# AlexGr5/StereoVision

Hardware: AMD Instinct MI355X
Metric: disparity frames/sec + HBM GB/s, 1920x1080 D=128 win=9, 1/2/4/8 GPU (higher is better)
Workload: dtype u8

## Files before the change

stereovision_amd/csrc/sv_capi.cpp:

```cpp
#include "sv_ctx.h"

namespace {
thread_local std::string g_err;
}

namespace svc {

int fail(int code, const std::string& msg) {
    g_err = msg;
    return code;
}

int hipfail(int e, const char* what) {
    return fail(SV_EHIP, std::string(what) + ": " + hipGetErrorString((hipError_t)e));
}

const std::string& last_error_msg() { return g_err; }

int check_image(const void* a, int H, int W) {
    if (!a || H <= 0 || W <= 0) return fail(SV_EINVAL, "null image or non-positive size");
    return 0;
}

int check_match(int H, int W, int min_disp, int num_disp, int win, int cost, sv::MatchPlan* plan) {
// ... 3 lines not shown
    if (min_disp < -4096 || min_disp > 4096) return fail(SV_EINVAL, "min_disp out of range");
    if (cost == SV_COST_SGBM) return 0;
    int rc = sv::plan_match(num_disp, win, cost, plan);
    if (rc == -34) return fail(SV_ERANGE, "cost range too large for the argmin key");
    if (rc != 0) return fail(SV_EINVAL, "unsupported (num_disp, win, cost)");
    return 0;
}

SgbmParams sgbm_reference_params(int win) {
    return {8 * 3 * win * win, 32 * 3 * win * win, 1, 63, 10, 100, 32};
}

int enqueue_speckles(sv_ctx* c, int16_t* d_img, int H, int W, int pitch, int new_val, int max_speckle_size,
                     int max_diff, hipStream_t s, int nf, long long fimg) {
    if (max_speckle_size <= 0) return 0;
    const size_t n = (size_t)H * W * (nf < 1 ? 1 : nf);
    SV_HIP(c->cc_parent.ensure(n * 4));
    SV_HIP(c->cc_size.ensure(n * 4));
    SV_LAUNCH(c, SV_K_SPECKLE, s,
              sv::launch_speckles(d_img, H, W, pitch, new_val, max_speckle_size, max_diff, c->cc_parent.as<int>(),
                                  c->cc_size.as<int>(), s, nf < 1 ? 1 : nf, fimg));
    return 0;
}

constexpr int kSgbmChunk = 32;
size_t sgbm_budget(int device) {
    static const long long env_gb = [] {
        const char* e = std::getenv("SV_SGBM_BUDGET_GB");
        return e ? std::atoll(e) : 0LL;
    }();
    if (env_gb > 0) return (size_t)env_gb << 30;
    size_t fr = 0, tot = 0;
    (void)device;
    if (hipMemGetInfo(&fr, &tot) != hipSuccess || fr == 0) return (size_t)8 << 30;
    return std::min<size_t>(fr / 4, (size_t)48 << 30);
}

int enqueue_sgbm(sv_ctx* c, const uint8_t* L, const uint8_t* R, int H, int W, int pitch, int min_disp,
                 int num_disp, int win, SgbmParams p, int16_t* out, int opitch, hipStream_t s, int nf,
                 long long fs_in, long long fs_out) {
    if (nf < 1) nf = 1;
    if (sv::sgbm_dp(num_disp) < 0) return fail(SV_EINVAL, "num_disp must be in [1, 512]");
    if (W > 16384) return fail(SV_EINVAL, "SGBM: width beyond 16384");
    if (p.P1 < 0 || p.P2 < 0) return fail(SV_EINVAL, "negative P1/P2");
    if (p.P2 <= p.P1) p.P2 = p.P1 + 1;
    if (p.P2 >= 349525) return fail(SV_ERANGE, "SGBM: P2 too large for the 32-bit argmin key");
    p.cap = (p.cap > 15 ? p.cap : 15) | 1;
    if (p.cap > 127) return fail(SV_EINVAL, "preFilterCap must be <= 127");
    sv::SgbmArgs a{};
    a.L = L;
    a.R = R;
    a.H = H;
    a.W = W;
    a.pitch = pitch;
    a.minD = min_disp;
    a.D = num_disp;
// ... 57 lines not shown
        const int n = std::min(chunk, nf - z0);
        a.L = L + z0 * fs_in;
        a.R = R + z0 * fs_in;
        a.out = out + z0 * fs_out;
        SV_LAUNCH(c, SV_K_SGBM, s, sv::launch_sgbm(a, n, s, c->sg_aux, c->sg_ev[0], c->sg_ev[1]));
        const int rc = enqueue_speckles(c, a.out, H, W, opitch, (min_disp - 1) * 16, p.speckle_win,
                                        16 * p.speckle_range, s, n, fs_out);
        if (rc) return rc;
    }
    return 0;
}

int enqueue_disparity(sv_ctx* c, const uint8_t* L, const uint8_t* R, int H, int W, int pitch,
                      int min_disp, int num_disp, int win, int cost, int row0, int row1,
                      int16_t* out, int opitch, hipStream_t s, int nf, long long fs_in,
                      long long fs_out) {
    sv::MatchPlan plan;
    int rc = check_match(H, W, min_disp, num_disp, win, cost, &plan);
    if (rc) return rc;
    if (row0 < 0) row0 = 0;
    if (row1 > H) row1 = H;
    if (row1 <= row0) return 0;
    if (cost == SV_COST_SGBM) {
        if (row0 != 0 || row1 != H) return fail(SV_EINVAL, "SGBM cannot compute a row band (use frames)");
        return enqueue_sgbm(c, L, R, H, W, pitch, min_disp, num_disp, win, sgbm_reference_params(win), out, opitch,
                            s, nf, fs_in, fs_out);
    }
    sv::MatchParams a{};
    a.L = L;
    a.R = R;
    a.H = H;
    a.W = W;
    a.pitch = pitch;
    a.minD = min_disp;
    a.D = num_disp;
    a.win = win;
    a.r = cost == SV_COST_HOG ? 0 : win / 2;
// ... 22 lines not shown
        SV_HIP(c->hog[0].ensure(hb));
        SV_HIP(c->hog[1].ensure(hb));
        SV_LAUNCH(c, SV_K_HOG, s,
                  sv::launch_hog_hist_pairs(L, R, H, W, pitch, win, row0, row1, c->hog[0].as<uint16_t>(),
                                            c->hog[1].as<uint16_t>(), a.nf, a.nf > 1 ? fs_in : 0, fh, s));
        a.HL = c->hog[0].as<uint16_t>();
        a.HR = c->hog[1].as<uint16_t>();
        a.fs_hist = a.nf > 1 ? fh : 0;
    }
    if (sv::ring_split(cost, win, num_disp) && a.X1 > a.X0) {
        const long long ke = sv::ring_split_elems(a.nf, fs_out, row1, opitch);
        SV_HIP(c->keys.ensure((size_t)(2 * ke) * sizeof(uint32_t)));
        a.keys = c->keys.as<uint32_t>();
        a.keys_stride = ke;
    }
    SV_LAUNCH(c, SV_K_MATCH, s, sv::launch_match(a, plan, cost, s));
    return 0;
}

int attach_lut(sv_ctx* c, sv::PostParams& pp, hipStream_t s, bool whole) {
    pp.lut_n = 0;
    pp.lut_shift = 0;
    if (pp.mode == SV_POST_NONE || pp.num_disp <= 0 || pp.num_disp > 512) return 0;
    sv_ctx::LutKey k;
    k.mode = pp.mode;
    k.min_disp = pp.min_disp;
    k.num_disp = pp.num_disp;
    k.m0 = (pp.min_disp - 1) * 16;
    k.n = whole ? pp.num_disp + 1 : (pp.num_disp + 1) * 16;
    k.minf = pp.minf;
    k.maxf = pp.maxf;
    k.rangef = pp.rangef;
    k.mdg = pp.min_disp_global;
    DevBuf& buf = whole ? c->lutw : c->lut;
    sv_ctx::LutKey& key = whole ? c->lutw_key : c->lut_key;
    hipEvent_t& ev = whole ? c->lutw_ev : c->lut_ev;
    hipStream_t& bs = whole ? c->lutw_stream : c->lut_stream;
    const size_t n = (size_t)k.n;
    float* la = buf.as<float>();
    if (!(k == key) || !ev) {
        SV_HIP(buf.ensure(n * (2 * sizeof(float) + 1)));
        la = buf.as<float>();
        if (!ev) SV_HIP(hipEventCreateWithFlags(&ev, hipEventDisableTiming));
        int e = sv::launch_post_lut(pp, k.m0, k.n, whole ? 16 : 1, la, reinterpret_cast<uint8_t*>(la + 2 * n), la + n,
                                    s);
        if (e) return hipfail(e, "launch_post_lut");
        SV_HIP(hipEventRecord(ev, s));
        key = k;
        bs = s;
    } else if (s != bs) {
        SV_HIP(hipStreamWaitEvent(s, ev, 0));
    }
    pp.lut_a = la;
    pp.lut_b = la + n;
    pp.lut_u8 = reinterpret_cast<const uint8_t*>(la + 2 * n);
    pp.lut_m0 = k.m0;
    pp.lut_n = k.n;
    pp.lut_shift = whole ? 4 : 0;
    return 0;
}

int attach_cmap(sv_ctx* c, sv::PostParams& pp, const uint8_t* table, uint8_t* d_bgr, hipStream_t s) {
    pp.out_bgr = nullptr;
    pp.cmap = nullptr;
    if (!d_bgr) return 0;
    if (!table) return fail(SV_EINVAL, "colormap output without a table");
    SV_HIP(c->cmap.ensure(256 * sizeof(uint32_t)));
    if (!c->cmap_valid || std::memcmp(c->cmap_host, table, 768) != 0) {
        uint32_t packed[256];
        for (int i = 0; i < 256; ++i)
            packed[i] = (uint32_t)table[3 * i] | ((uint32_t)table[3 * i + 1] << 8) | ((uint32_t)table[3 * i + 2] << 16);
        SV_HIP(hipMemcpyAsync(c->cmap.p, packed, sizeof(packed), hipMemcpyHostToDevice, s));
        SV_HIP(hipStreamSynchronize(s));
// ... 275 lines not shown
    SV_ENTER(c);
    if (slot < 0 || slot >= 16 || !c->wev[slot]) return fail(SV_EINVAL, "event slot never recorded");
    SV_HIP(hipStreamWaitEvent(pick(c, stream), c->wev[slot], 0));
    return 0;
}

int sv_release_scratch(sv_ctx* c) {
    SV_ENTER(c);
    SV_HIP(hipStreamSynchronize(c->stream));
    if (c->sg_aux) SV_HIP(hipStreamSynchronize(c->sg_aux));
    DevBuf* bufs[] = {&c->img[0], &c->img[1], &c->gray[0], &c->gray[1], &c->d16, &c->fa, &c->fb, &c->fc,
                      &c->u8, &c->harris, &c->hog[0], &c->hog[1], &c->fin, &c->sg_hsum, &c->sg_c,
                      &c->sg_l, &c->sg_lt, &c->sg_band, &c->sg_rec, &c->cc_parent, &c->cc_size, &c->m16,
                      &c->gm16, &c->keys};
    for (auto* b : bufs) b->release();
    return 0;
}

int sv_synchronize(sv_ctx* c) {
    SV_ENTER(c);
    SV_HIP(hipStreamSynchronize(c->stream));
    return 0;
}

void* sv_stream(sv_ctx* c) { return c ? static_cast<void*>(c->stream) : nullptr; }

int sv_plan(int num_disp, int win, int cost, int* dpl, int* lpg, int* lds_bytes) {
    sv::MatchPlan p;
    int rc = sv::plan_match(num_disp, win, cost, &p);
    if (rc == -34) return fail(SV_ERANGE, "cost range too large for the argmin key");
// ... 121 lines not shown
```

stereovision_amd/csrc/sv_capi_dev.cpp:

```cpp
#include "sv_ctx.h"

extern "C" {

int sv_gray_dev(sv_ctx* c, const uint8_t* d_bgr, int H, int W, int pitch, uint8_t* d_gray, void* stream) {
    SV_ENTER(c);
    if (check_image(d_bgr, H, W) || !d_gray) return fail(SV_EINVAL, "bad gray arguments");
    hipStream_t s = pick(c, stream);
    SV_LAUNCH(c, SV_K_GRAY, s, sv::launch_gray(d_bgr, H, W, pitch, d_gray, s));
    return 0;
}

int sv_disparity_dev(sv_ctx* c, const uint8_t* d_left, const uint8_t* d_right, int H, int W, int pitch,
                     int min_disp, int num_disp, int win, int cost, int row0, int row1, int16_t* d_disp16,
                     int out_pitch, void* stream) {
    SV_ENTER(c);
    if (check_image(d_left, H, W) || check_image(d_right, H, W) || !d_disp16)
        return fail(SV_EINVAL, "bad disparity arguments");
    if (pitch < W || out_pitch < W) return fail(SV_EINVAL, "pitch smaller than width");
    hipStream_t s = pick(c, stream);
    SV_SCRATCH(c, s);
    return enqueue_disparity(c, d_left, d_right, H, W, pitch, min_disp, num_disp, win, cost, row0, row1,
                             d_disp16, out_pitch, s);
}

// ... 68 lines not shown
    if (median && out->harris && check_image(d_left, H, W)) return fail(SV_EINVAL, "Harris needs the left frames");
    if (pitch < W) return fail(SV_EINVAL, "pitch smaller than width");
    if (n_frames > 1 && frame_stride < (int64_t)pitch * H) return fail(SV_EINVAL, "frame stride smaller than a frame");
    if ((long long)H * W >= (1LL << 30)) return fail(SV_EINVAL, "frame too large for the median kernel");
    if (n_frames == 0) return 0;
    hipStream_t s = pick(c, stream);
    SV_SCRATCH(c, s);
    const long long fs = (long long)H * W;
    int16_t* d16 = d_disp16;
    if (!d16) {
        SV_HIP(c->d16.ensure((size_t)n_frames * fs * sizeof(int16_t)));
        d16 = c->d16.as<int16_t>();
    }
    if (match) {
        const int rc = enqueue_disparity(c, d_left, d_right, H, W, pitch, min_disp, num_disp, win, cost, 0, H, d16, W,
                                         s, n_frames, frame_stride, fs);
        if (rc) return rc;
    }
    if (!median) return 0;
    sv::PostParams pp;
    float* disp = nullptr;
    int rc = map_out_post(c, out, min_disp, num_disp, cost, true, s, &pp, &disp);
    if (rc) return rc;
    const long long fin = n_frames > 1 ? frame_stride : 0;
    if (out->harris && (W < 8 || H < 8)) {
        SV_LAUNCH(c, SV_K_MEDIAN, s, sv::launch_median_i16(d16, H, W, 0, H, disp, pp, s, n_frames, fs, fs));
        SV_LAUNCH(c, SV_K_HARRIS, s, sv::launch_harris(d_left, H, W, pitch, out->harris, s, n_frames, fin, fs));
        return 0;
    }
    sv::HarrisParams hp{d_left, pitch, fin, out->harris, fs, 0, 0};
    SV_LAUNCH(c, SV_K_MEDIAN, s,
              sv::launch_median_i16(d16, H, W, 0, H, disp, pp, s, n_frames, fs, fs, out->harris ? &hp : nullptr));
    return 0;
}

int sv_harris_dev(sv_ctx* c, const uint8_t* d_gray, int H, int W, int pitch, float* d_out, void* stream) {
    SV_ENTER(c);
    if (check_image(d_gray, H, W) || !d_out) return fail(SV_EINVAL, "bad harris arguments");
// ... 990 lines not shown
    SV_ENTER(c);
    if (!d_img || H <= 0 || W <= 0 || pitch < W) return fail(SV_EINVAL, "bad speckle-filter arguments");
    hipStream_t s = pick(c, stream);
    SV_SCRATCH(c, s);
    return enqueue_speckles(c, d_img, H, W, pitch, new_val, max_speckle_size, max_diff, s);
}

int sv_filter_speckles(sv_ctx* c, int16_t* img, int H, int W, int new_val, int max_speckle_size, int max_diff) {
    SV_ENTER(c);
    SV_SCRATCH(c, c->stream);
    if (!img || H <= 0 || W <= 0) return fail(SV_EINVAL, "bad speckle-filter arguments");
    const size_t bytes = (size_t)H * W * sizeof(int16_t);
    SV_HIP(c->d16.ensure(bytes));
    SV_HIP(c->hin.ensure(bytes));
    std::memcpy(c->hin.p, img, bytes);
    SV_HIP(hipMemcpyAsync(c->d16.p, c->hin.p, bytes, hipMemcpyHostToDevice, c->stream));
    const int rc = enqueue_speckles(c, c->d16.as<int16_t>(), H, W, W, new_val, max_speckle_size, max_diff, c->stream);
    if (rc) return rc;
    Out o[] = {{img, c->d16.p, bytes}};
    return collect(c, o, 1);
}


}
```

stereovision_amd/csrc/sv_ctx.h:

```cpp
#pragma once
#include <cstdio>
#include <cstdlib>
#include <algorithm>
#include <chrono>
#include <cstring>
#include <map>
#include <mutex>
#include <thread>
#include <new>
#include <string>
#include <vector>

#include "sv_internal.h"
#include "sv_pool.h"
#include "../../include/stereovision_amd.h"

namespace svc {
int fail(int code, const std::string& msg);
int hipfail(int e, const char* what);
const std::string& last_error_msg();
}
using svc::fail;
using svc::hipfail;

// ... 5 lines not shown

#define SV_LAUNCH(ctx, kid, stream, call)                          \
    do {                                                           \
        (ctx)->prof_begin((kid), (stream));                        \
        int e_ = (call);                                           \
        if (e_ != 0) {                                             \
            (ctx)->prof_abort();                                   \
            return hipfail(e_, #call);                             \
        }                                                          \
        (ctx)->prof_end((stream));                                 \
    } while (0)

struct DevBuf {
    void* p = nullptr;
    size_t cap = 0;
    hipError_t ensure(size_t n) {
        if (n <= cap) return hipSuccess;
        if (p) (void)hipFree(p);
        p = nullptr;
        cap = 0;
        hipError_t e = hipMalloc(&p, n);
        if (e == hipSuccess) cap = n;
        return e;
    }
    void release() {
        if (p) (void)hipFree(p);
        p = nullptr;
        cap = 0;
    }
    hipError_t ensure_zeroed(size_t n) {
        if (n <= cap) return hipSuccess;
        hipError_t e = ensure(n);
        if (e == hipSuccess) e = hipMemset(p, 0, cap);
        if (e == hipSuccess) e = hipDeviceSynchronize();
        return e;
    }
    template <class T> T* as() const { return static_cast<T*>(p); }
};

struct HostBuf {
// ... 52 lines not shown
        bool operator==(const LutKey& o) const {
            return mode == o.mode && min_disp == o.min_disp && num_disp == o.num_disp && m0 == o.m0 &&
                   n == o.n && std::memcmp(&minf, &o.minf, sizeof(float)) == 0 &&
                   std::memcmp(&maxf, &o.maxf, sizeof(float)) == 0 &&
                   std::memcmp(&rangef, &o.rangef, sizeof(float)) == 0 &&
                   std::memcmp(&mdg, &o.mdg, sizeof(float)) == 0;
        }
    } lut_key, hl_key;
    hipEvent_t lut_ev = nullptr;
    hipStream_t lut_stream = nullptr;
    DevBuf lutw;
    LutKey lutw_key;
    hipEvent_t lutw_ev = nullptr;
    hipStream_t lutw_stream = nullptr;
    HostBuf hin, hout;
    hipStream_t scr_stream = nullptr;
    hipEvent_t scr_ev = nullptr;
    hipEvent_t xev = nullptr;
    hipEvent_t sev = nullptr;
    hipEvent_t gev = nullptr;
    hipEvent_t wev[16] = {};
    bool prof = false;
    std::vector<EvPair> pending;
    std::vector<hipEvent_t> pool;
    double acc_ms[SV_NKERNELS] = {};
    long long cnt[SV_NKERNELS] = {};
    EvPair cur{};
    bool cur_open = false;
    EvPair region{};
    bool region_open = false;
// ... 62 lines not shown
struct SgbmParams {
    int P1, P2, disp12, cap, uniq, speckle_win, speckle_range;
};
SgbmParams sgbm_reference_params(int win);

int check_image(const void* a, int H, int W);
int check_match(int H, int W, int min_disp, int num_disp, int win, int cost, sv::MatchPlan* plan);
int enqueue_speckles(sv_ctx* c, int16_t* d_img, int H, int W, int pitch, int new_val, int max_speckle_size,
                     int max_diff, hipStream_t s, int nf = 1, long long fimg = 0);
int enqueue_sgbm(sv_ctx* c, const uint8_t* L, const uint8_t* R, int H, int W, int pitch, int min_disp,
                 int num_disp, int win, SgbmParams p, int16_t* out, int opitch, hipStream_t s, int nf = 1,
                 long long fs_in = 0, long long fs_out = 0);
int enqueue_disparity(sv_ctx* c, const uint8_t* L, const uint8_t* R, int H, int W, int pitch,
                      int min_disp, int num_disp, int win, int cost, int row0, int row1,
                      int16_t* out, int opitch, hipStream_t s, int nf = 1, long long fs_in = 0,
                      long long fs_out = 0);
int attach_lut(sv_ctx* c, sv::PostParams& pp, hipStream_t s, bool whole = false);
int attach_cmap(sv_ctx* c, sv::PostParams& pp, const uint8_t* table, uint8_t* d_bgr, hipStream_t s);
sv::PostParams make_post(int mode, float minf, float maxf, float rangef, float mdg, int min_disp,
                         int num_disp, float* a, uint8_t* u8, float* b);

int map_out_post(sv_ctx* c, const sv_map_out* out, int min_disp, int num_disp, int cost, bool allow_harris,
                 hipStream_t s, sv::PostParams* pp, float** disp);

struct MapOut {
    int fmt = 0;
    void* map = nullptr;
    int d8_base = 0;
    size_t el() const { return fmt == SV_MAP_D8 ? 1 : 2; }
};
int check_map(int fmt, const void* map, int cost, int num_disp);
// ... 57 lines not shown
```

stereovision_amd/csrc/sv_image.hip:

```cpp
#include <cstdlib>
#include <cstring>
#include <type_traits>
#include "sv_internal.h"
#include "sv_median_net.h"

namespace sv {
namespace {

__device__ __forceinline__ int clampi(int v, int lo, int hi) { return min(max(v, lo), hi); }
__device__ __forceinline__ int refl101(int i, int n) {
    if (n == 1) return 0;
    i = i < 0 ? -i : i;
    return i >= n ? 2 * (n - 1) - i : i;
}

__global__ void k_gray(const uint8_t* __restrict__ bgr, int H, int W, int pitch,
                       uint8_t* __restrict__ gray) {
    const int x = blockIdx.x * blockDim.x + threadIdx.x;
    const int y = blockIdx.y;
    if (x >= W) return;
    const uint8_t* p = bgr + (size_t)y * pitch + 3 * x;
    const int v = p[0] * 1868 + p[1] * 9617 + p[2] * 4899 + (1 << 13);
    gray[(size_t)y * W + x] = (uint8_t)(v >> 14);
}
// ... 619 lines not shown
    return *reinterpret_cast<T*>(reinterpret_cast<B*>(base) + (uint32_t)(i * (uint32_t)sizeof(T)));
}

__device__ __forceinline__ PostVals post_median(const PostParams& pp, int mv) {
    const uint32_t dm = (uint32_t)(mv - pp.lut_m0);
    const uint32_t li = dm >> pp.lut_shift;
    if (li < (uint32_t)pp.lut_n && (dm & ((1u << pp.lut_shift) - 1u)) == 0) {
        PostVals o;
        o.a = at(pp.lut_a, li);
        o.u = at(pp.lut_u8, li);
        o.b = pp.mode == POST_SCALED ? at(pp.lut_b, li) : 0.0f;
        return o;
    }
    return post_vals(pp, (float)mv / 16.0f);
}

__global__ __launch_bounds__(256) void k_post_m16(const int16_t* __restrict__ in, long long n,
                                                  float* __restrict__ disp, PostParams pp) {
    const long long i0 = ((long long)blockIdx.x * 256 + threadIdx.x) * 8;
    if (i0 >= n) return;
    const bool vec = i0 + 8 <= n && ((((uintptr_t)in) & 15) | (((uintptr_t)disp | (uintptr_t)pp.out_a |
                                                                  (uintptr_t)pp.out_b) & 15) |
                                     ((uintptr_t)pp.out_u8 & 7)) == 0;
    if (vec) {
        const uint4 raw = *reinterpret_cast<const uint4*>(in + i0);
        const uint32_t w[4] = {raw.x, raw.y, raw.z, raw.w};
        int mv[8];
#pragma unroll
        for (int q = 0; q < 4; ++q) {
            mv[2 * q] = (int)(int16_t)(w[q] & 0xFFFFu);
// ... 21 lines not shown
            b[1] = make_float4(o[4].b, o[5].b, o[6].b, o[7].b);
        }
        return;
    }
    for (long long i = i0; i < i0 + 8 && i < n; ++i) {
        const int mv = (int)in[i];
        if (disp) disp[i] = (float)mv / 16.0f;
        if (pp.mode == POST_NONE) continue;
        const PostVals o = post_median(pp, mv);
        pp.out_a[i] = o.a;
        pp.out_u8[i] = o.u;
        if (pp.mode == POST_SCALED) pp.out_b[i] = o.b;
    }
}

template <int HF>
__global__ __launch_bounds__(256) void k_median_i16(const int16_t* __restrict__ in, int H, int W,
                                                    int row0, int row1, float* __restrict__ disp,
                                                    PostParams pp, long long fs_in, long long fs_out,
                                                    HarrisParams hp) {
    if (HF != 0 && (int)blockIdx.x >= hp.mbx) {
        const int w = (int)(blockIdx.x - hp.mbx) * 4 + (int)(threadIdx.x >> 6);
        const int y0 = row0 + (int)blockIdx.y * MQ_H;
        if constexpr (HF == 2) {
            const int x0 = w * 248;
            if (x0 < W && y0 < row1)
                harris_wave4<MQ_H, 4>(hp.g + blockIdx.z * hp.fs_in, H, W, hp.pitch, hp.out + blockIdx.z * hp.fs_out,
                                      x0, y0, threadIdx.x & 63);
        } else {
            const int x0 = w * 60;
            if (x0 < W && y0 < row1)
// ... 146 lines not shown
            for (int i = 0; i < 5; ++i) r = __builtin_elementwise_min(r, __builtin_elementwise_max(cw[w][i], u[4 - i]));
            m[w] = r;
        }
        const uint32_t a0 = __builtin_bit_cast(uint32_t, m[0]), a1 = __builtin_bit_cast(uint32_t, m[1]);
        mp[h] = (a0 & 0xFFFFu) | (a1 << 16);
        mp[h + 2] = (a0 >> 16) | (a1 & 0xFFFF0000u);
    }
    static_assert(sizeof(srt) >= MQ_H * (MQ_W / 2) * sizeof(uint32_t), "med must fit in srt");
    auto med = reinterpret_cast<uint32_t (*)[MQ_W / 2]>(&srt[0][0][0]);
    __syncthreads();
    med[tb][tx >> 1] = mp[0];
    med[tb + 1][tx >> 1] = mp[1];
    med[tb + 2][tx >> 1] = mp[2];
    med[tb + 3][tx >> 1] = mp[3];
    __syncthreads();
#pragma unroll
    for (int pass = 0; pass < 2; ++pass) {
        const int r = (int)(threadIdx.x >> 5) + 8 * pass, c4 = (int)(threadIdx.x & 31) * 4;
        const int y = y0 + r, x = x0 + c4;
        if (y >= row1 || x >= W) continue;
        const uint2 raw = *reinterpret_cast<const uint2*>(&med[r][c4 >> 1]);
        const int mv[4] = {(int)(int16_t)(raw.x & 0xFFFF), (int)(int16_t)(raw.x >> 16),
                           (int)(int16_t)(raw.y & 0xFFFF), (int)(int16_t)(raw.y >> 16)};
        const uint32_t i = (uint32_t)y * W + x;
        const bool vec = x + 3 < W && (W & 3) == 0 &&
                         (((uintptr_t)disp | (uintptr_t)pp.out_a | (uintptr_t)pp.out_b) & 15) == 0 &&
                         (((uintptr_t)pp.out_u8 | (uintptr_t)pp.out_bgr | (uintptr_t)pp.out_d8) & 3) == 0 &&
                         ((uintptr_t)pp.out_m16 & 7) == 0;
        if (vec) {
            if (disp)
                at(reinterpret_cast<float4*>(disp), i >> 2) =
                    make_float4((float)mv[0] / 16.0f, (float)mv[1] / 16.0f, (float)mv[2] / 16.0f, (float)mv[3] / 16.0f);
            if (pp.out_m16) at(reinterpret_cast<uint2*>(pp.out_m16), i >> 2) = raw;
            if (pp.out_d8)
                at(reinterpret_cast<uint32_t*>(pp.out_d8), i >> 2) =
                    (uint32_t)(uint8_t)((mv[0] >> 4) - pp.d8_base) | ((uint32_t)(uint8_t)((mv[1] >> 4) - pp.d8_base) << 8) |
                    ((uint32_t)(uint8_t)((mv[2] >> 4) - pp.d8_base) << 16) |
                    ((uint32_t)(uint8_t)((mv[3] >> 4) - pp.d8_base) << 24);
            if (pp.mode == POST_NONE) continue;
            PostVals o[4];
#pragma unroll
            for (int q = 0; q < 4; ++q) o[q] = post_median(pp, mv[q]);
            at(reinterpret_cast<float4*>(pp.out_a), i >> 2) = make_float4(o[0].a, o[1].a, o[2].a, o[3].a);
            at(reinterpret_cast<uint32_t*>(pp.out_u8), i >> 2) =
                (uint32_t)o[0].u | ((uint32_t)o[1].u << 8) | ((uint32_t)o[2].u << 16) | ((uint32_t)o[3].u << 24);
            if (pp.mode == POST_SCALED)
                at(reinterpret_cast<float4*>(pp.out_b), i >> 2) = make_float4(o[0].b, o[1].b, o[2].b, o[3].b);
            if (pp.out_bgr) {
                const uint32_t c0 = pp.cmap[o[0].u], c1 = pp.cmap[o[1].u], c2 = pp.cmap[o[2].u],
                               c3 = pp.cmap[o[3].u];
                uint32_t* d = &at(reinterpret_cast<uint32_t*>(pp.out_bgr), 3 * (i >> 2));
                d[0] = c0 | (c1 << 24);
                d[1] = (c1 >> 8) | (c2 << 16);
                d[2] = (c2 >> 16) | (c3 << 8);
            }
            continue;
        }
#pragma unroll
        for (int q = 0; q < 4; ++q) {
            if (x + q >= W) break;
            if (disp) at(disp, i + q) = (float)mv[q] / 16.0f;
            if (pp.out_m16) at(pp.out_m16, i + q) = (int16_t)mv[q];
            if (pp.out_d8) at(pp.out_d8, i + q) = (uint8_t)((mv[q] >> 4) - pp.d8_base);
            if (pp.mode == POST_NONE) continue;
            const PostVals o = post_median(pp, mv[q]);
            at(pp.out_a, i + q) = o.a;
            at(pp.out_u8, i + q) = o.u;
            if (pp.mode == POST_SCALED) at(pp.out_b, i + q) = o.b;
            if (pp.out_bgr) {
                const uint32_t c = pp.cmap[o.u];
                uint8_t* d = &at(pp.out_bgr, 3 * (i + q));
                d[0] = (uint8_t)c;
                d[1] = (uint8_t)(c >> 8);
                d[2] = (uint8_t)(c >> 16);
            }
        }
    }
}

__global__ __launch_bounds__(256) void k_median_f32(const float* __restrict__ in, int H, int W,
// ... 142 lines not shown
    if (row1 <= row0 || nf <= 0) return 0;
    if ((long long)H * W >= (1LL << 30)) return (int)hipErrorInvalidValue;
    HarrisParams hp{};
    hp.mbx = (W + MQ_W - 1) / MQ_W;
    int hbx = 0;
    if (harris && harris->g) {
        hp = *harris;
        hp.mbx = (W + MQ_W - 1) / MQ_W;
        static const bool med4 = [] {
            const char* e = std::getenv("SV_HARRIS_MED4");
            return !(e && e[0] == '0');
        }();
        hp.form = (med4 && W >= 256) ? 1 : 0;
        hbx = hp.form ? ((W + 247) / 248 + 3) / 4 : ((W + 59) / 60 + 3) / 4;
    }
    void (*fn)(const int16_t*, int, int, int, int, float*, PostParams, long long, long long, HarrisParams) =
        hbx == 0 ? k_median_i16<0> : hp.form ? k_median_i16<2> : k_median_i16<1>;
    hipLaunchKernelGGL(fn, dim3(hp.mbx + hbx, (row1 - row0 + MQ_H - 1) / MQ_H, nf),
                       dim3(256), 0, s, in, H, W, row0, row1, disp, pp, fs_in, fs_out, hp);
    return (int)hipGetLastError();
}

int launch_post_m16(const int16_t* in, long long n, float* disp, const PostParams& pp, hipStream_t s) {
    if (n <= 0) return 0;
    const long long blocks = (n + 8 * 256 - 1) / (8 * 256);
    if (blocks > 0x7FFFFFFFLL) return (int)hipErrorInvalidValue;
    hipLaunchKernelGGL(k_post_m16, dim3((unsigned)blocks), dim3(256), 0, s, in, n, disp, pp);
    return (int)hipGetLastError();
}

int launch_median_f32(const float* in, int H, int W, float* out, hipStream_t s) {
    hipLaunchKernelGGL(k_median_f32, dim3((W + MT_W - 1) / MT_W, (H + MT_H - 1) / MT_H), dim3(256),
// ... 26 lines not shown
```

stereovision_amd/csrc/sv_internal.h:

```cpp
#pragma once
#include <hip/hip_runtime.h>
#include <stdint.h>

#include <string>

struct sv_comm;

namespace sv {

__device__ __forceinline__ void sad_u32_acc(uint32_t& a, uint32_t b, uint32_t c) {
    asm("v_sad_u32 %0, %0, %1, %2" : "+v"(a) : "v"(b), "v"(c));
}

int set_error(int code, const std::string& msg);

int comm_group_start();
int comm_group_end();
int comm_send(sv_comm* c, const void* buf, size_t bytes, int peer, hipStream_t s);
int comm_recv(sv_comm* c, void* buf, size_t bytes, int peer, hipStream_t s);
int comm_rank(const sv_comm* c);
int comm_size(const sv_comm* c);
int comm_device(const sv_comm* c);

enum Cost { COST_SAD = 0, COST_SSD = 1, COST_HOG = 2, COST_SGBM = 3 };
// ... 15 lines not shown
    int minD, D, r;
    int win;
    int X0, X1;
    int row0, row1;
    int lpg, lpg_log2, dbits;
    int16_t* out;
    int opitch;
    int nf;
    long long fs_in, fs_out, fs_hist;
    uint32_t pad_key;
    int segm;
    unsigned* work_ctr;
    int xcd_map;
    uint32_t* keys;
    long long keys_stride;
};

int plan_match(int num_disp, int win, int cost, MatchPlan* plan);
uint64_t max_cost(int win, int cost);
size_t match_lds_bytes(const MatchPlan& p, int r, int cost);
int launch_match(const MatchParams& a, const MatchPlan& p, int cost, hipStream_t s);
bool ring_split(int cost, int win, int num_disp);
bool ring_ssd(int cost, int win, int num_disp);
bool ssd_mfma(int cost, int win, int num_disp);
bool ssd_mfma_fits(const MatchParams& a, int cost);
int launch_ssd_mfma(const MatchParams& a, hipStream_t s);
long long ring_split_elems(int nf, long long fs_out, int row1, int opitch);
int launch_fill_i16(int16_t* out, int opitch, int H, int W, int16_t v, hipStream_t s);

int launch_gray(const uint8_t* bgr, int H, int W, int pitch, uint8_t* gray, hipStream_t s);
// ... 116 lines not shown
    float minf, maxf, rangef, min_disp_global;
    int min_disp, num_disp;
    float* out_a;
    uint8_t* out_u8;
    float* out_b;
    uint8_t* out_bgr;
    const uint32_t* cmap;
    int16_t* out_m16;
    uint8_t* out_d8;
    int d8_base;
    const float* lut_a;
    const uint8_t* lut_u8;
    const float* lut_b;
    int lut_m0, lut_n;
    int lut_shift;
};
struct HarrisParams {
    const uint8_t* g;
    int pitch;
    long long fs_in;
    float* out;
    long long fs_out;
    int mbx;
    int form;
};
int launch_median_i16(const int16_t* in, int H, int W, int row0, int row1, float* disp,
                      const PostParams& pp, hipStream_t s, int nf = 1, long long fs_in = 0,
                      long long fs_out = 0, const HarrisParams* harris = nullptr);
int launch_median_f32(const float* in, int H, int W, float* out, hipStream_t s);
int launch_post_m16(const int16_t* in, long long n, float* disp, const PostParams& pp, hipStream_t s);
int launch_post(const float* disp, int n, const PostParams& pp, hipStream_t s);
// ... 5 lines not shown
```

stereovision_amd/csrc/sv_match.hip:

```cpp
#include "sv_internal.h"
#include "sv_xcd.h"

#include <algorithm>
#include <cstdlib>
#include <vector>
#include <cstdio>
#include <type_traits>

namespace sv {
namespace {

constexpr int COST_SAD4 = 4;

__host__ __device__ __forceinline__ int seg_width(int lpg, int dpl, int sm = 4) { return (sm * lpg + dpl - 1) / dpl * dpl; }
__host__ __device__ __forceinline__ int wave_cols(int lpg, int dpl, int sm = 4) { return (64 / lpg) * seg_width(lpg, dpl, sm); }
int seg_mult(int kind, int r) {
    static const int sm4 = [] {
        const char* e = std::getenv("SV_SAD4_SEG");
        const int v = e ? std::atoi(e) : 0;
        return v >= 1 && v <= 8 ? v : 0;
    }();
    if (kind != COST_SAD4) return 4;
    if (sm4) return sm4;
    return (2 * r - 2 + 3) / 4 <= 2 ? 4 : 2;
// ... 162 lines not shown
__device__ __forceinline__ void transpose4(uint32_t a, uint32_t b, uint32_t c, uint32_t d, uint32_t (&o)[4]) {
    const uint32_t t0 = __builtin_amdgcn_perm(b, a, 0x05010400u);
    const uint32_t t1 = __builtin_amdgcn_perm(b, a, 0x07030602u);
    const uint32_t t2 = __builtin_amdgcn_perm(d, c, 0x05010400u);
    const uint32_t t3 = __builtin_amdgcn_perm(d, c, 0x07030602u);
    o[0] = __builtin_amdgcn_perm(t2, t0, 0x05040100u);
    o[1] = __builtin_amdgcn_perm(t2, t0, 0x07060302u);
    o[2] = __builtin_amdgcn_perm(t3, t1, 0x05040100u);
    o[3] = __builtin_amdgcn_perm(t3, t1, 0x07060302u);
}

template <int R>
__device__ __forceinline__ void sad4_group_words(const uint32_t (&rw)[2 * R + 4],
                                                 uint32_t (&w)[PackCfg<COST_SAD4, R>::NW][4]) {
    constexpr int NC = PackCfg<COST_SAD4, R>::NW - 4, NCR = 2 * R - 2;
#pragma unroll
    for (int m = 0; m < NC; ++m) {
        uint32_t d[4];
#pragma unroll
        for (int t = 0; t < 4; ++t) d[t] = 4 * m + t < NCR ? rw[3 + 4 * m + t] : 0u;
        transpose4(d[0], d[1], d[2], d[3], w[m]);
    }
#pragma unroll
    for (int q = 0; q < 4; ++q) {
        uint32_t d[3];
        int n = 0;
#pragma unroll
        for (int j = q; j <= 2; ++j) d[n++] = rw[j];
#pragma unroll
        for (int j = 2 * R + 1; j <= 2 * R + q; ++j) d[n++] = rw[j];
        transpose4(d[0], d[1], d[2], 0u, w[NC + q]);
    }
}

template <int COST, int ND>
__device__ __forceinline__ void build_group(const MatchParams& a, const uint8_t* img, int cg, int y,
                                            uint32_t (&w)[PackCfg<COST, ND>::NW][4]) {
    const int r = COST == COST_SAD4 ? ND : a.r;
    auto row = [&](int j) -> uint32_t {
        const int yy = clampi(y - r + j, 0, a.H - 1);
        return *reinterpret_cast<const uint32_t*>(img + (size_t)yy * a.pitch + cg);
    };
    if constexpr (COST == COST_SAD4) {
        uint32_t rw[2 * ND + 4];
#pragma unroll
        for (int j = 0; j < 2 * ND + 4; ++j) rw[j] = row(j);
// ... 56 lines not shown
                for (int i = 0; i < 8; ++i) v[i] = i < NW ? w[i < NW ? i : 0][k] : 0u;
                put<COST, ND>(base + (right ? rslot(idx, c0, DPL) : idx), v);
            }
        } else {
#pragma unroll
            for (int k = 0; k < 4; ++k) {
                const int idx = cg + k - cfirst;
                if (idx < 0 || idx >= n) continue;
                build_pack<COST, ND>(a, img, nullptr, cg + k, y, base + (right ? rslot(idx, c0, DPL) : idx));
            }
        }
    }
    }
}

template <int R, int MF, int DPL>
__device__ __forceinline__ void build_ring_packs(const MatchParams& a, int y, int cL0, int NL, int cR0,
                                                 int NRlog, int c0, PackOut<COST_SAD4, R> Lp,
                                                 PackOut<COST_SAD4, R> Rp, int lane) {
    constexpr int NW = PackCfg<COST_SAD4, R>::NW, NRW = 2 * R + 4;
    const bool aligned = ((reinterpret_cast<uintptr_t>(a.L) | reinterpret_cast<uintptr_t>(a.R) |
                           (uintptr_t)a.pitch) & 3u) == 0;
    const bool near = (long long)a.H * (long long)a.pitch < 0x7FFFFFFFLL;
    if (!aligned || !near) {
        build_all_packs<COST_SAD4, R, DPL>(a, y, cL0, NL, cR0, NRlog, c0, Lp, Rp, lane);
        return;
    }
    const auto lsrc = __builtin_amdgcn_make_buffer_rsrc(const_cast<uint8_t*>(a.L), 0, 0x7FFFFFFF, 0x00020000);
    const auto rsrc = __builtin_amdgcn_make_buffer_rsrc(const_cast<uint8_t*>(a.R), 0, 0x7FFFFFFF, 0x00020000);
    const int aL = cL0 & ~3, aR = cR0 & ~3;
    const int gL = (cL0 + NL - aL + 3) >> 2, gR = (cR0 + NRlog - aR + 3) >> 2;
    const int G = gL + gR;
    int roff[NRW];
#pragma unroll
    for (int j = 0; j < NRW; ++j) roff[j] = clampi(y - R + j, 0, a.H - 1) * a.pitch;
    for (int g0 = 0; g0 < G; g0 += 64 * MF) {
        uint32_t rw[MF][NRW];
#pragma unroll
        for (int m = 0; m < MF; ++m) {
            const int gi = g0 + lane + 64 * m;
            const bool right = gi >= gL;
            const int cg = right ? aR + 4 * (gi - gL) : aL + 4 * gi;
            const bool in = gi < G && cg >= 0 && cg + 4 <= a.W;
            if (in && !right) {
#pragma unroll
                for (int j = 0; j < NRW; ++j) rw[m][j] = __builtin_amdgcn_raw_buffer_load_b32(lsrc, cg, roff[j], 0);
            }
            if (in && right) {
#pragma unroll
                for (int j = 0; j < NRW; ++j) rw[m][j] = __builtin_amdgcn_raw_buffer_load_b32(rsrc, cg, roff[j], 0);
            }
        }
#pragma unroll
        for (int m = 0; m < MF; ++m) {
            const int gi = g0 + lane + 64 * m;
            if (gi >= G) continue;
            const bool right = gi >= gL;
            const int cg = right ? aR + 4 * (gi - gL) : aL + 4 * gi;
            const int cfirst = right ? cR0 : cL0, n = right ? NRlog : NL;
            const PackOut<COST_SAD4, R> base = right ? Rp : Lp;
            if (cg >= 0 && cg + 4 <= a.W) {
                uint32_t w[NW][4];
                sad4_group_words<R>(rw[m], w);
#pragma unroll
                for (int k = 0; k < 4; ++k) {
                    const int idx = cg + k - cfirst;
                    if (idx < 0 || idx >= n) continue;
                    uint32_t v[8];
#pragma unroll
                    for (int i = 0; i < 8; ++i) v[i] = i < NW ? w[i < NW ? i : 0][k] : 0u;
                    put<COST_SAD4, R>(base + (right ? rslot(idx, c0, DPL) : idx), v);
                }
            } else {
#pragma unroll
                for (int k = 0; k < 4; ++k) {
                    const int idx = cg + k - cfirst;
                    if (idx < 0 || idx >= n) continue;
                    build_pack<COST_SAD4, R>(a, right ? a.R : a.L, nullptr, cg + k, y,
                                             base + (right ? rslot(idx, c0, DPL) : idx));
                }
            }
        }
    }
}

template <int COST, int ND, int DPL>
// ... 357 lines not shown
    constexpr int LPG = LPGT;
    const int S = a.segm;
    const int WC = (64 / LPG) * S;
    constexpr bool SADU = PK || R <= 5;
    constexpr int M = SADU ? W2 + 1 : W2;
    constexpr int U = M % 4 == 0 ? M : M % 2 == 0 ? 2 * M : 4 * M;
    constexpr int NCH = U / 4;
    const int Tn = (S + 2 * R + 3) & ~3;
    const int nit = (Tn + U - 1) / U;
    const int e0 = (nit * U - Tn) >> 2;
    const int NL = WC - S + Tn + 1;
    const int NRlog = WC - S + Tn + 4 * LPG;
    constexpr int c0 = 1;
    const int NRphys = NRlog + (NRlog + c0) / RG_DPL + 1;
    uint4* wbase = smem + (LDSMIN ? RING_SCRATCH_BYTES / 16 : 0);
    typename P::CT* cbase = reinterpret_cast<typename P::CT*>(wbase + (size_t)(NL + NRphys));
    const PackOut<COST_SAD4, R> Lw{wbase, cbase};
    const PackOut<COST_SAD4, R> Rw{wbase + NL, cbase + NL};
    const PackPtr<COST_SAD4, R> Lp{Lw.x, Lw.c};
    const PackPtr<COST_SAD4, R> Rp{Rw.x, Rw.c};

    const int y = a.row0 + by * 4;
    const int yc = min(y, a.row1 - 1);
    const int xw = a.X0 + bx * WC;
    const int cL0 = xw - R;
    const int cR0 = cL0 - a.minD - (4 * LPG - 1);
    build_ring_packs<R, 3, RG_DPL>(a, yc, cL0, NL, cR0, NRlog, c0, Lw, Rw, lane);

    if (!KEYS && bx == 0) {
        const int16_t inv = (int16_t)((a.minD - 1) * 16);
#pragma unroll
        for (int q = 0; q < 4; ++q) {
            if (y + q >= a.row1) break;
            int16_t* orow = a.out + (size_t)(y + q) * a.opitch;
            for (int x = lane; x < a.X0; x += 64) orow[x] = inv;
            for (int x = a.X1 + lane; x < a.W; x += 64) orow[x] = inv;
        }
    }
    __syncthreads();
    if (y >= a.row1) return;

    const int g = lane / LPG;
    const int l = lane & (LPG - 1);
    const int xs = xw + g * S;
// ... 362 lines not shown
    const int G = 64 / lpg;
    int best = 8;
    long long best_cost = -1;
    for (int S = 8; S <= 1024; S += 4) {
        if (S > 8 && ring_lds_bytes(lpg, S, r, ldsmin) > 20 * 1024) break;
        const long long cost = (long long)((band + G * S - 1) / (G * S)) * ((S + 2 * r + 3) & ~3);
        if (best_cost < 0 || cost <= best_cost) { best = S; best_cost = cost; }
    }
    return best;
}
size_t ring_lds_bytes(int lpg, int seg, int r, bool ldsmin) {
    const int wc = (64 / lpg) * seg;
    const int tn = (seg + 2 * r + 3) & ~3;
    const int nl = wc - seg + tn + 1, nr = wc - seg + tn + 4 * lpg;
    const int nrp = nr + (nr + 1) / RG_DPL + 1;
    return (size_t)(nl + nrp) * (r <= 3 ? 20 : r <= 5 ? 24 : 28) + (ldsmin ? RING_SCRATCH_BYTES : 0);
}

template <int R, int LPG, bool KEYS, bool SSD>
int launch_ring_rl(const MatchParams& a, size_t lds, hipStream_t s) {
    static const bool defer = [] {
        const char* e = std::getenv("SV_RING_DEFER");
        return !(e && e[0] == '0');
    }();
    void (*fn)(MatchParams);
    if constexpr (SSD) fn = k_match_ring<R, LPG, R != 5, false, true>;
    else if constexpr (KEYS) fn = k_match_ring<R, LPG, R != 5, true>;
    else fn = (defer && R != 5) ? k_match_ring<R, LPG, R != 5, false> : k_match_ring<R, LPG, false, false>;
    if constexpr (R == 4 && LPG == 32 && !KEYS && !SSD) {
        if (ring_ldsmin(LPG, R, KEYS, SSD)) fn = k_match_ring<R, LPG, false, false, false, true>;
    }
// ... 213 lines not shown
```

Baseline: 31770.

## Skip repeated margin fills, use unchecked whole LUT, and streamline ring pack building

Tracks whether the invalid-disparity margins of the internal d16 buffer were already written, keyed on buffer identity, generation and geometry. When the key matches, the ring match kernel skips refilling those margins. The median kernel gains a whole-LUT variant that masks the index instead of range checking, backed by a padded LUT allocation, and its vector-store check is hoisted out of the loop. The SAD4 word transpose is rebuilt with byte-permute instructions, and right-ring slot stores use a computed base with padded LDS. The risks are stale margins if another writer reaches d16 without invalidating the key, and slightly more LDS per block.

```diff
diff --git a/stereovision_amd/csrc/sv_capi.cpp b/stereovision_amd/csrc/sv_capi.cpp
--- a/stereovision_amd/csrc/sv_capi.cpp
+++ b/stereovision_amd/csrc/sv_capi.cpp
@@ -41,6 +41,7 @@
 int enqueue_speckles(sv_ctx* c, int16_t* d_img, int H, int W, int pitch, int new_val, int max_speckle_size,
                      int max_diff, hipStream_t s, int nf, long long fimg) {
     if (max_speckle_size <= 0) return 0;
+    c->scratch_written(d_img);
     const size_t n = (size_t)H * W * (nf < 1 ? 1 : nf);
     SV_HIP(c->cc_parent.ensure(n * 4));
     SV_HIP(c->cc_size.ensure(n * 4));
@@ -67,6 +68,7 @@
                  int num_disp, int win, SgbmParams p, int16_t* out, int opitch, hipStream_t s, int nf,
                  long long fs_in, long long fs_out) {
     if (nf < 1) nf = 1;
+    c->scratch_written(out);
     if (sv::sgbm_dp(num_disp) < 0) return fail(SV_EINVAL, "num_disp must be in [1, 512]");
     if (W > 16384) return fail(SV_EINVAL, "SGBM: width beyond 16384");
     if (p.P1 < 0 || p.P2 < 0) return fail(SV_EINVAL, "negative P1/P2");
@@ -154,13 +156,15 @@
 int enqueue_disparity(sv_ctx* c, const uint8_t* L, const uint8_t* R, int H, int W, int pitch,
                       int min_disp, int num_disp, int win, int cost, int row0, int row1,
                       int16_t* out, int opitch, hipStream_t s, int nf, long long fs_in,
-                      long long fs_out) {
+                      long long fs_out, bool track_margins) {
     sv::MatchPlan plan;
     int rc = check_match(H, W, min_disp, num_disp, win, cost, &plan);
     if (rc) return rc;
     if (row0 < 0) row0 = 0;
     if (row1 > H) row1 = H;
     if (row1 <= row0) return 0;
+    const sv_ctx::MarginKey had = c->d16_margins;
+    c->scratch_written(out);
     if (cost == SV_COST_SGBM) {
         if (row0 != 0 || row1 != H) return fail(SV_EINVAL, "SGBM cannot compute a row band (use frames)");
         return enqueue_sgbm(c, L, R, H, W, pitch, min_disp, num_disp, win, sgbm_reference_params(win), out, opitch,
@@ -213,13 +217,31 @@
         a.keys = c->keys.as<uint32_t>();
         a.keys_stride = ke;
     }
+    sv_ctx::MarginKey key;
+    if (track_margins && out == c->d16.as<int16_t>() && row0 == 0 && row1 == H) {
+        key.valid = true;
+        key.p = c->d16.p;
+        key.gen = c->d16.gen;
+        key.H = H;
+        key.W = W;
+        key.opitch = opitch;
+        key.X0 = a.X0;
+        key.X1 = a.X1;
+        key.min_disp = min_disp;
+        key.nf = a.nf;
+        key.fs_out = fs_out;
+        a.margins_done = had.covers(key) ? 1 : 0;
+        if (a.margins_done) key = had;
+    }
     SV_LAUNCH(c, SV_K_MATCH, s, sv::launch_match(a, plan, cost, s));
+    if (key.valid) c->d16_margins = key;
     return 0;
 }
 
 int attach_lut(sv_ctx* c, sv::PostParams& pp, hipStream_t s, bool whole) {
     pp.lut_n = 0;
     pp.lut_shift = 0;
+    pp.lut_cap = 0;
     if (pp.mode == SV_POST_NONE || pp.num_disp <= 0 || pp.num_disp > 512) return 0;
     sv_ctx::LutKey k;
     k.mode = pp.mode;
@@ -238,7 +260,7 @@
     const size_t n = (size_t)k.n;
     float* la = buf.as<float>();
     if (!(k == key) || !ev) {
-        SV_HIP(buf.ensure(n * (2 * sizeof(float) + 1)));
+        SV_HIP(buf.ensure(whole ? (n + sv::kLutWholeSpan) * 2 * sizeof(float) : n * (2 * sizeof(float) + 1)));
         la = buf.as<float>();
         if (!ev) SV_HIP(hipEventCreateWithFlags(&ev, hipEventDisableTiming));
         int e = sv::launch_post_lut(pp, k.m0, k.n, whole ? 16 : 1, la, reinterpret_cast<uint8_t*>(la + 2 * n), la + n,
@@ -256,6 +278,7 @@
     pp.lut_m0 = k.m0;
     pp.lut_n = k.n;
     pp.lut_shift = whole ? 4 : 0;
+    pp.lut_cap = whole ? k.n + sv::kLutWholeSpan : k.n;
     return 0;
 }
 
@@ -561,6 +584,7 @@
                       &c->sg_l, &c->sg_lt, &c->sg_band, &c->sg_rec, &c->cc_parent, &c->cc_size, &c->m16,
                       &c->gm16, &c->keys};
     for (auto* b : bufs) b->release();
+    c->d16_margins.valid = false;
     return 0;
 }
 
diff --git a/stereovision_amd/csrc/sv_capi_dev.cpp b/stereovision_amd/csrc/sv_capi_dev.cpp
--- a/stereovision_amd/csrc/sv_capi_dev.cpp
+++ b/stereovision_amd/csrc/sv_capi_dev.cpp
@@ -106,7 +106,7 @@
     }
     if (match) {
         const int rc = enqueue_disparity(c, d_left, d_right, H, W, pitch, min_disp, num_disp, win, cost, 0, H, d16, W,
-                                         s, n_frames, frame_stride, fs);
+                                         s, n_frames, frame_stride, fs, !d_disp16);
         if (rc) return rc;
     }
     if (!median) return 0;
@@ -114,6 +114,8 @@
     float* disp = nullptr;
     int rc = map_out_post(c, out, min_disp, num_disp, cost, true, s, &pp, &disp);
     if (rc) return rc;
+    pp.lut_unchecked = match && cost != SV_COST_SGBM && pp.lut_shift == 4 && pp.lut_m0 == (min_disp - 1) * 16 &&
+                       pp.lut_n == num_disp + 1;
     const long long fin = n_frames > 1 ? frame_stride : 0;
     if (out->harris && (W < 8 || H < 8)) {
         SV_LAUNCH(c, SV_K_MEDIAN, s, sv::launch_median_i16(d16, H, W, 0, H, disp, pp, s, n_frames, fs, fs));
@@ -1134,6 +1136,7 @@
     SV_HIP(c->d16.ensure(bytes));
     SV_HIP(c->hin.ensure(bytes));
     std::memcpy(c->hin.p, img, bytes);
+    c->scratch_written(c->d16.p);
     SV_HIP(hipMemcpyAsync(c->d16.p, c->hin.p, bytes, hipMemcpyHostToDevice, c->stream));
     const int rc = enqueue_speckles(c, c->d16.as<int16_t>(), H, W, W, new_val, max_speckle_size, max_diff, c->stream);
     if (rc) return rc;
diff --git a/stereovision_amd/csrc/sv_ctx.h b/stereovision_amd/csrc/sv_ctx.h
--- a/stereovision_amd/csrc/sv_ctx.h
+++ b/stereovision_amd/csrc/sv_ctx.h
@@ -43,8 +43,10 @@
 struct DevBuf {
     void* p = nullptr;
     size_t cap = 0;
+    unsigned long long gen = 0;
     hipError_t ensure(size_t n) {
         if (n <= cap) return hipSuccess;
+        ++gen;
         if (p) (void)hipFree(p);
         p = nullptr;
         cap = 0;
@@ -53,6 +55,7 @@
         return e;
     }
     void release() {
+        ++gen;
         if (p) (void)hipFree(p);
         p = nullptr;
         cap = 0;
@@ -135,6 +138,23 @@
     hipEvent_t lutw_ev = nullptr;
     hipStream_t lutw_stream = nullptr;
     HostBuf hin, hout;
+    struct MarginKey {
+        bool valid = false;
+        const void* p = nullptr;
+        unsigned long long gen = 0;
+        int H = 0, W = 0, opitch = 0, X0 = 0, X1 = 0, min_disp = 0, nf = 0;
+        long long fs_out = 0;
+        bool covers(const MarginKey& o) const {
+            return valid && p == o.p && gen == o.gen && H == o.H && W == o.W && opitch == o.opitch &&
+                   X0 == o.X0 && X1 == o.X1 && min_disp == o.min_disp && nf >= o.nf &&
+                   (o.nf <= 1 || fs_out == o.fs_out);
+        }
+    } d16_margins;
+    void scratch_written(const void* out) {
+        const char* b = static_cast<const char*>(d16.p);
+        const char* o = static_cast<const char*>(out);
+        if (b && o >= b && o < b + d16.cap) d16_margins.valid = false;
+    }
     hipStream_t scr_stream = nullptr;
     hipEvent_t scr_ev = nullptr;
     hipEvent_t xev = nullptr;
@@ -227,7 +247,7 @@
 int enqueue_disparity(sv_ctx* c, const uint8_t* L, const uint8_t* R, int H, int W, int pitch,
                       int min_disp, int num_disp, int win, int cost, int row0, int row1,
                       int16_t* out, int opitch, hipStream_t s, int nf = 1, long long fs_in = 0,
-                      long long fs_out = 0);
+                      long long fs_out = 0, bool track_margins = false);
 int attach_lut(sv_ctx* c, sv::PostParams& pp, hipStream_t s, bool whole = false);
 int attach_cmap(sv_ctx* c, sv::PostParams& pp, const uint8_t* table, uint8_t* d_bgr, hipStream_t s);
 sv::PostParams make_post(int mode, float minf, float maxf, float rangef, float mdg, int min_disp,
diff --git a/stereovision_amd/csrc/sv_image.hip b/stereovision_amd/csrc/sv_image.hip
--- a/stereovision_amd/csrc/sv_image.hip
+++ b/stereovision_amd/csrc/sv_image.hip
@@ -657,6 +657,14 @@
     }
     return post_vals(pp, (float)mv / 16.0f);
 }
+__device__ __forceinline__ PostVals post_median_whole(const PostParams& pp, int mv) {
+    const uint32_t li = ((uint32_t)(mv - pp.lut_m0) >> 4) & (uint32_t)(kLutWholeSpan - 1);
+    PostVals o;
+    o.a = at(pp.lut_a, li);
+    o.u = at(pp.lut_u8, li);
+    o.b = pp.mode == POST_SCALED ? at(pp.lut_b, li) : 0.0f;
+    return o;
+}
 
 __global__ __launch_bounds__(256) void k_post_m16(const int16_t* __restrict__ in, long long n,
                                                   float* __restrict__ disp, PostParams pp) {
@@ -708,7 +716,7 @@
     }
 }
 
-template <int HF>
+template <int HF, bool WH>
 __global__ __launch_bounds__(256) void k_median_i16(const int16_t* __restrict__ in, int H, int W,
                                                     int row0, int row1, float* __restrict__ disp,
                                                     PostParams pp, long long fs_in, long long fs_out,
@@ -885,6 +893,11 @@
     med[tb + 2][tx >> 1] = mp[2];
     med[tb + 3][tx >> 1] = mp[3];
     __syncthreads();
+    auto post = [&](int mv) { return WH ? post_median_whole(pp, mv) : post_median(pp, mv); };
+    const bool vec = (W & 3) == 0 &&
+                     (((uintptr_t)disp | (uintptr_t)pp.out_a | (uintptr_t)pp.out_b) & 15) == 0 &&
+                     (((uintptr_t)pp.out_u8 | (uintptr_t)pp.out_bgr | (uintptr_t)pp.out_d8) & 3) == 0 &&
+                     ((uintptr_t)pp.out_m16 & 7) == 0;
 #pragma unroll
     for (int pass = 0; pass < 2; ++pass) {
         const int r = (int)(threadIdx.x >> 5) + 8 * pass, c4 = (int)(threadIdx.x & 31) * 4;
@@ -894,10 +907,6 @@
         const int mv[4] = {(int)(int16_t)(raw.x & 0xFFFF), (int)(int16_t)(raw.x >> 16),
                            (int)(int16_t)(raw.y & 0xFFFF), (int)(int16_t)(raw.y >> 16)};
         const uint32_t i = (uint32_t)y * W + x;
-        const bool vec = x + 3 < W && (W & 3) == 0 &&
-                         (((uintptr_t)disp | (uintptr_t)pp.out_a | (uintptr_t)pp.out_b) & 15) == 0 &&
-                         (((uintptr_t)pp.out_u8 | (uintptr_t)pp.out_bgr | (uintptr_t)pp.out_d8) & 3) == 0 &&
-                         ((uintptr_t)pp.out_m16 & 7) == 0;
         if (vec) {
             if (disp)
                 at(reinterpret_cast<float4*>(disp), i >> 2) =
@@ -911,7 +920,7 @@
             if (pp.mode == POST_NONE) continue;
             PostVals o[4];
 #pragma unroll
-            for (int q = 0; q < 4; ++q) o[q] = post_median(pp, mv[q]);
+            for (int q = 0; q < 4; ++q) o[q] = post(mv[q]);
             at(reinterpret_cast<float4*>(pp.out_a), i >> 2) = make_float4(o[0].a, o[1].a, o[2].a, o[3].a);
             at(reinterpret_cast<uint32_t*>(pp.out_u8), i >> 2) =
                 (uint32_t)o[0].u | ((uint32_t)o[1].u << 8) | ((uint32_t)o[2].u << 16) | ((uint32_t)o[3].u << 24);
@@ -934,7 +943,7 @@
             if (pp.out_m16) at(pp.out_m16, i + q) = (int16_t)mv[q];
             if (pp.out_d8) at(pp.out_d8, i + q) = (uint8_t)((mv[q] >> 4) - pp.d8_base);
             if (pp.mode == POST_NONE) continue;
-            const PostVals o = post_median(pp, mv[q]);
+            const PostVals o = post(mv[q]);
             at(pp.out_a, i + q) = o.a;
             at(pp.out_u8, i + q) = o.u;
             if (pp.mode == POST_SCALED) at(pp.out_b, i + q) = o.b;
@@ -1107,8 +1116,11 @@
         hp.form = (med4 && W >= 256) ? 1 : 0;
         hbx = hp.form ? ((W + 247) / 248 + 3) / 4 : ((W + 59) / 60 + 3) / 4;
     }
+    const bool wh = pp.lut_unchecked && pp.mode != POST_NONE && pp.lut_shift == 4 && pp.lut_n > 0 &&
+                    pp.lut_cap >= kLutWholeSpan;
     void (*fn)(const int16_t*, int, int, int, int, float*, PostParams, long long, long long, HarrisParams) =
-        hbx == 0 ? k_median_i16<0> : hp.form ? k_median_i16<2> : k_median_i16<1>;
+        wh ? (hbx == 0 ? k_median_i16<0, true> : hp.form ? k_median_i16<2, true> : k_median_i16<1, true>)
+           : (hbx == 0 ? k_median_i16<0, false> : hp.form ? k_median_i16<2, false> : k_median_i16<1, false>);
     hipLaunchKernelGGL(fn, dim3(hp.mbx + hbx, (row1 - row0 + MQ_H - 1) / MQ_H, nf),
                        dim3(256), 0, s, in, H, W, row0, row1, disp, pp, fs_in, fs_out, hp);
     return (int)hipGetLastError();
diff --git a/stereovision_amd/csrc/sv_internal.h b/stereovision_amd/csrc/sv_internal.h
--- a/stereovision_amd/csrc/sv_internal.h
+++ b/stereovision_amd/csrc/sv_internal.h
@@ -53,6 +53,7 @@
     int xcd_map;
     uint32_t* keys;
     long long keys_stride;
+    int margins_done;
 };
 
 int plan_match(int num_disp, int win, int cost, MatchPlan* plan);
@@ -199,7 +200,10 @@
     const float* lut_b;
     int lut_m0, lut_n;
     int lut_shift;
-};
+    int lut_unchecked;
+    int lut_cap;
+};
+constexpr int kLutWholeSpan = 4096;
 struct HarrisParams {
     const uint8_t* g;
     int pitch;
diff --git a/stereovision_amd/csrc/sv_match.hip b/stereovision_amd/csrc/sv_match.hip
--- a/stereovision_amd/csrc/sv_match.hip
+++ b/stereovision_amd/csrc/sv_match.hip
@@ -200,22 +200,32 @@
 __device__ __forceinline__ void sad4_group_words(const uint32_t (&rw)[2 * R + 4],
                                                  uint32_t (&w)[PackCfg<COST_SAD4, R>::NW][4]) {
     constexpr int NC = PackCfg<COST_SAD4, R>::NW - 4, NCR = 2 * R - 2;
+    static_assert(NCR % 4 == 0 || NCR % 4 == 2, "the common block's last word holds 4 or 2 rows");
 #pragma unroll
     for (int m = 0; m < NC; ++m) {
-        uint32_t d[4];
-#pragma unroll
-        for (int t = 0; t < 4; ++t) d[t] = 4 * m + t < NCR ? rw[3 + 4 * m + t] : 0u;
-        transpose4(d[0], d[1], d[2], d[3], w[m]);
-    }
-#pragma unroll
-    for (int q = 0; q < 4; ++q) {
-        uint32_t d[3];
-        int n = 0;
-#pragma unroll
-        for (int j = q; j <= 2; ++j) d[n++] = rw[j];
-#pragma unroll
-        for (int j = 2 * R + 1; j <= 2 * R + q; ++j) d[n++] = rw[j];
-        transpose4(d[0], d[1], d[2], 0u, w[NC + q]);
+        const int b = 3 + 4 * m;
+        if (4 * m + 4 <= NCR) {
+            transpose4(rw[b], rw[b + 1], rw[b + 2], rw[b + 3], w[m]);
+        } else {
+#pragma unroll
+            for (int k = 0; k < 4; ++k)
+                w[m][k] = __builtin_amdgcn_perm(rw[b + 1], rw[b], 0x0c0c0400u + 0x0101u * (uint32_t)k);
+        }
+    }
+    constexpr int P = 2 * R + 1;
+    const uint32_t pa[2] = {__builtin_amdgcn_perm(rw[2], rw[1], 0x05010400u),
+                            __builtin_amdgcn_perm(rw[2], rw[1], 0x07030602u)};
+    const uint32_t pb[2] = {__builtin_amdgcn_perm(rw[P + 1], rw[P], 0x05010400u),
+                            __builtin_amdgcn_perm(rw[P + 1], rw[P], 0x07030602u)};
+#pragma unroll
+    for (int k = 0; k < 4; ++k) {
+        const uint32_t p0 = 4u + 2u * (k & 1), p1 = p0 + 1u, s = (uint32_t)k;
+        const uint32_t row_pair = 0x0c000000u | (p1 << 16) | (p0 << 8) | s;
+        const uint32_t pair_row = 0x0c000000u | (s << 16) | (p1 << 8) | p0;
+        w[NC + 0][k] = __builtin_amdgcn_perm(pa[k >> 1], rw[0], row_pair);
+        w[NC + 1][k] = __builtin_amdgcn_perm(pa[k >> 1], rw[P], pair_row);
+        w[NC + 2][k] = __builtin_amdgcn_perm(pb[k >> 1], rw[2], row_pair);
+        w[NC + 3][k] = __builtin_amdgcn_perm(pb[k >> 1], rw[P + 2], pair_row);
     }
 }
 
@@ -302,6 +312,8 @@
     }
 }
 
+constexpr int RING_PAD_F = 3, RING_PAD_M = 4, RING_PAD_B = 3;
+constexpr int RING_PAD = RING_PAD_F + RING_PAD_M + RING_PAD_B;
 template <int R, int MF, int DPL>
 __device__ __forceinline__ void build_ring_packs(const MatchParams& a, int y, int cL0, int NL, int cR0,
                                                  int NRlog, int c0, PackOut<COST_SAD4, R> Lp,
@@ -322,6 +334,7 @@
     int roff[NRW];
 #pragma unroll
     for (int j = 0; j < NRW; ++j) roff[j] = clampi(y - R + j, 0, a.H - 1) * a.pitch;
+    static_assert(DPL == 4, "a 4-column group meets one slot gap at a wave-uniform column");
     for (int g0 = 0; g0 < G; g0 += 64 * MF) {
         uint32_t rw[MF][NRW];
 #pragma unroll
@@ -350,14 +363,21 @@
             if (cg >= 0 && cg + 4 <= a.W) {
                 uint32_t w[NW][4];
                 sad4_group_words<R>(rw[m], w);
-#pragma unroll
-                for (int k = 0; k < 4; ++k) {
-                    const int idx = cg + k - cfirst;
-                    if (idx < 0 || idx >= n) continue;
+                auto store = [&](const PackOut<COST_SAD4, R> gb, int k, int slot) {
                     uint32_t v[8];
 #pragma unroll
                     for (int i = 0; i < 8; ++i) v[i] = i < NW ? w[i < NW ? i : 0][k] : 0u;
-                    put<COST_SAD4, R>(base + (right ? rslot(idx, c0, DPL) : idx), v);
+                    put<COST_SAD4, R>(gb + slot, v);
+                };
+                if (right) {
+                    const int d = aR - cR0;
+                    const PackOut<COST_SAD4, R> gb = Rp + (d + ((cg - aR) >> 2) * (DPL + 1));
+#pragma unroll
+                    for (int k = 0; k < 4; ++k) store(gb, k, k + ((d + k + c0 + DPL) >> 2) - 1);
+                } else {
+                    const PackOut<COST_SAD4, R> gb = Lp + (cg - cL0);
+#pragma unroll
+                    for (int k = 0; k < 4; ++k) store(gb, k, k);
                 }
             } else {
 #pragma unroll
@@ -745,9 +765,9 @@
     constexpr int c0 = 1;
     const int NRphys = NRlog + (NRlog + c0) / RG_DPL + 1;
     uint4* wbase = smem + (LDSMIN ? RING_SCRATCH_BYTES / 16 : 0);
-    typename P::CT* cbase = reinterpret_cast<typename P::CT*>(wbase + (size_t)(NL + NRphys));
-    const PackOut<COST_SAD4, R> Lw{wbase, cbase};
-    const PackOut<COST_SAD4, R> Rw{wbase + NL, cbase + NL};
+    typename P::CT* cbase = reinterpret_cast<typename P::CT*>(wbase + (size_t)(NL + NRphys + RING_PAD));
+    const PackOut<COST_SAD4, R> Lw{wbase + RING_PAD_F, cbase + RING_PAD_F};
+    const PackOut<COST_SAD4, R> Rw{wbase + NL + RING_PAD_F + RING_PAD_M, cbase + NL + RING_PAD_F + RING_PAD_M};
     const PackPtr<COST_SAD4, R> Lp{Lw.x, Lw.c};
     const PackPtr<COST_SAD4, R> Rp{Rw.x, Rw.c};
 
@@ -758,7 +778,7 @@
     const int cR0 = cL0 - a.minD - (4 * LPG - 1);
     build_ring_packs<R, 3, RG_DPL>(a, yc, cL0, NL, cR0, NRlog, c0, Lw, Rw, lane);
 
-    if (!KEYS && bx == 0) {
+    if (!KEYS && bx == 0 && !a.margins_done) {
         const int16_t inv = (int16_t)((a.minD - 1) * 16);
 #pragma unroll
         for (int q = 0; q < 4; ++q) {
@@ -1151,7 +1171,7 @@
     const int tn = (seg + 2 * r + 3) & ~3;
     const int nl = wc - seg + tn + 1, nr = wc - seg + tn + 4 * lpg;
     const int nrp = nr + (nr + 1) / RG_DPL + 1;
-    return (size_t)(nl + nrp) * (r <= 3 ? 20 : r <= 5 ? 24 : 28) + (ldsmin ? RING_SCRATCH_BYTES : 0);
+    return (size_t)(nl + nrp + RING_PAD) * (r <= 3 ? 20 : r <= 5 ? 24 : 28) + (ldsmin ? RING_SCRATCH_BYTES : 0);
 }
 
 template <int R, int LPG, bool KEYS, bool SSD>
```

New measurement: 32310, median of 6. 1.02x the previous value.
